# mokemokechicken/reversi-alpha-zero

Hardware: NVIDIA H100
Metric: self_play_games_per_sec (higher is better)
Workload: dtype f16

## Files before the change

### include/rz_engine.h

```cpp
#ifndef RZ_ENGINE_H
#define RZ_ENGINE_H

#include <stddef.h>
#include <stdint.h>

#ifdef __cplusplus
extern "C" {
#endif

#define RZ_OK 0
#define RZ_EINVAL (-1)
#define RZ_ECUDA (-2)
#define RZ_ENOMEM (-3)
#define RZ_ESTATE (-4)
#define RZ_ECAPACITY (-5)
#define RZ_EIO (-6)

#define RZ_ABI_VERSION 2

int rz_abi_version(void);
const char* rz_last_error(void);
int rz_device_count(int* count);


// ... 89 lines not shown
    int32_t start_rethinking_turn;
    int32_t allowed_resign_turn;
    int32_t use_resign_threshold;
    int32_t share_mtcs_info;
    int32_t eval_mode;
    int32_t net_impl;
    int32_t max_plies;
    int32_t warm_start;
    int32_t overlap_groups;
    int32_t max_sims_per_wave;
    int32_t use_solver_turn;
    int32_t use_solver_turn_in_simulation;
    int32_t reset_mtcs_info_per_game;
    int32_t max_searches_per_game;
    int32_t arena_simulation_num;
    float c_puct;
    float noise_eps;
    float dirichlet_alpha;
    float resign_threshold;
    float disable_resignation_rate;
    uint64_t seed;
    uint64_t first_game_id;
    uint64_t game_id_stride;
    uint64_t max_games;
} rz_engine_cfg;

typedef struct rz_ply {
    uint64_t own, enemy;
    int32_t n_visit[64];
    int16_t action;
// ... 22 lines not shown
    uint8_t pad[2];
    int32_t table_nodes;
    int32_t pad2;
} rz_game;

typedef struct rz_stats {
    uint64_t games_started, games_finished;
    uint64_t expansions;
    uint64_t simulations;
    uint64_t waves;
    uint64_t plies;
    uint64_t nn_launches, mcts_launches;
    uint64_t max_nodes_used, max_edges_used;
    double nn_ms, mcts_ms;
    double run_ms;
} rz_stats;

int rz_engine_create(const rz_engine_cfg* cfg, rz_net* net , int device,
                     rz_engine** out);
int rz_engine_destroy(rz_engine* e);
int rz_engine_run(rz_engine* e, uint64_t finished_target, uint64_t max_waves);
int rz_engine_poll(rz_engine* e, rz_game* games, size_t game_cap, size_t* n_games, rz_ply* plies, size_t ply_cap,
                   size_t* n_plies);
int rz_engine_stats(rz_engine* e, rz_stats* out);
int rz_engine_set_max_games(rz_engine* e, uint64_t max_games);
int rz_engine_set_warm_start_profile(rz_engine* e, const float* weight, int n);
int rz_engine_set_simulation_num(rz_engine* e, int32_t sims);
int rz_engine_set_second_net(rz_engine* e, rz_net* net_b, int enable);
int rz_engine_set_resign_threshold(rz_engine* e, int use_resign_threshold, float resign_threshold);
int rz_engine_search_root(rz_engine* e, uint64_t own, uint64_t enemy, int player, int slot, int keep_tree,
                          int32_t* n_visit, float* w_sum);

int rz_write_play_data(const char* path, const rz_game* games, size_t n_games, const rz_ply* plies,
                       int save_policy_of_tau_1, int change_tau_turn, size_t* n_records);

typedef struct rz_play_row {
    uint64_t own, enemy;
    int32_t n_visit[64];
    int32_t z;
// ... 78 lines not shown
```

### reversi-alpha-zero_b200/csrc/rz_engine.cu

```cuda
#include <deque>
#include <mutex>
#include <new>
#include <vector>
#include <stdlib.h>
#include <string.h>
#include "rz_bitboard.cuh"
#include "rz_net.cuh"
#include "rz_solver.cuh"

namespace rz {
namespace solver {
constexpr int kBlockThreads = 128;
__global__ void __launch_bounds__(kBlockThreads) solve_active_kernel(SolveCtx* __restrict__ ctx, const uint32_t* __restrict__ active,
                                                                     const uint32_t* __restrict__ n_active, uint32_t* __restrict__ next,
                                                                     uint32_t* __restrict__ n_next, u64* tt_base, long long budget_ns) {
    const uint32_t n = *n_active;
    if (n == 0) return;
    const uint32_t tid = blockIdx.x * blockDim.x + threadIdx.x, total = gridDim.x * blockDim.x, n_warps = total >> 5;
    const long long deadline = global_ns() + budget_ns;
    const TT tt{tt_base + (size_t)tid * kTtEntries * kTtWordsPerEntry};
    for (uint32_t r = (tid & 31u) * n_warps + (tid >> 5); r < n; r += total) {
        const uint32_t idx = active[r];
        if (!solve_advance(ctx + idx, tt, deadline)) next[atomicAdd(n_next, 1u)] = idx;
    }
// ... 57 lines not shown
    u64 games_played;
    uint32_t gen;
    uint32_t n_nodes, n_edges;
    uint32_t n_expand, n_rootsel, n_sims, sims_started, sims_target;
    uint32_t ply;
    uint8_t phase, tl, log_sel, enable_resign;
    uint8_t resigned_mask, search_only, n_pending, n_parked;
    uint8_t pending[kMaxK], parked[kMaxK];
    u64 root_own, root_enemy;
    uint8_t root_pid, black_net, cur_net;
    uint8_t root_req;
    uint32_t ply_waves;
    uint32_t n_solves, n_searched_plies;
};

struct Status {
    unsigned long long games_started, games_finished, expansions, simulations, plies, idle_slots;
    unsigned long long max_nodes, max_edges;
    int error;
    int pad;
};

struct DevCfg {
    int G, S, K, vl, change_tau_turn, thinking_loop, required_visit, start_rethinking_turn, allowed_resign_turn;
    int use_resign, share, max_plies, warm_start, sims_cap, two_nets, solver_turn, solver_sim_turn, keep_games;
    float c_puct, noise_eps, alpha, resign_threshold, disable_resignation_rate;
    u64 seed, first_game_id, game_id_stride, max_games;
    uint32_t nodes_cap, edges_cap, hash_cap;
    float warm_cdf[60];
    float warm_waves[60];
};

struct DevPtrs {
    Slot* slots;
    Descent* desc;
    uint32_t* hash;
    Node* nodes;
    Edge* edges;
    rz_ply* plies;
    rz_game* mail_hdr;
    uint8_t* mail_flag;
    Status* status;
    uint32_t* batch_count;
    u64* batch_own;
    u64* batch_enemy;
    float* policy;
    float* value;
    solver::SolveCtx* sctx;
    uint32_t* sactive;
    uint32_t* solve_count;
    float* keep_policy;
    float* keep_value;
    u64* solver_tt;
};

__device__ __forceinline__ uint32_t hash_key(u64 own, u64 enemy, uint32_t kpid) {
    u64 h = own * 0x9E3779B97F4A7C15ULL ^ (enemy + 0x7F4A7C15ULL) * 0xC2B2AE3D27D4EB4FULL ^ (u64)kpid * 0x165667B19E3779F9ULL;
    h ^= h >> 29; h *= 0xBF58476D1CE4E5B9ULL; h ^= h >> 32;
    return (uint32_t)h;
}

#include "rz_engine_warp.cuh"

__global__ void fake_eval_kernel(const u64* __restrict__ own, const u64* __restrict__ enemy, const uint32_t* __restrict__ count,
                                 float* __restrict__ policy, float* __restrict__ value, float sign) {
    const uint32_t n = *count;
    for (uint32_t i = blockIdx.x * blockDim.x + threadIdx.x; i < n * 64; i += gridDim.x * blockDim.x) {
        policy[i] = 1.0f / 64.0f;
        if ((i & 63) == 0) value[i >> 6] = sign * ((float)(popc64(own[i >> 6]) - popc64(enemy[i >> 6])) / 64.0f);
    }
}

__global__ void init_slots_kernel(const DevCfg c, const DevPtrs p) {
    const int s = blockIdx.x * blockDim.x + threadIdx.x;
    if (s >= c.G) return;
// ... 61 lines not shown
    size_t solver_tt_words_per_group;
    int solve_parity[2];
    long long solver_budget_ns;
    void* arena[32];
    int n_arena;
    Status* h_status;
    uint8_t* h_flags;
    uint64_t waves, nn_launches, mcts_launches;
    uint64_t finished_total;
    std::deque<FinishedGame> queue;
    std::mutex queue_mutex;
    cudaEvent_t ev[2 * 3 * 8];
    cudaEvent_t ev_run[3];
    int ev_used;
    double nn_ms, mcts_ms, run_ms;
};

static int collect_timing(rz_engine* e) {
    for (int g = 0; g < e->n_groups; ++g)
        for (int i = 0; i < e->ev_used; ++i) {
            float a = 0.f, b = 0.f;
            cudaEvent_t* ev = e->ev + (g * 8 + i) * 3;
            RZ_CUDA_TRY(cudaEventElapsedTime(&a, ev[0], ev[1]));
            RZ_CUDA_TRY(cudaEventElapsedTime(&b, ev[1], ev[2]));
            e->mcts_ms += a; e->nn_ms += b;
        }
    e->ev_used = 0;
    return RZ_OK;
}

static int dev_alloc(rz_engine* e, void** ptr, size_t bytes, bool zero) {
// ... 25 lines not shown
                                            cudaMemcpyDeviceToHost, e->stream));
        RZ_CUDA_TRY(cudaMemsetAsync(e->dp.mail_flag + i, 0, 1, e->stream));
        RZ_CUDA_TRY(cudaStreamSynchronize(e->stream));
        {
            std::lock_guard<std::mutex> lock(e->queue_mutex);
            e->queue.push_back(std::move(fg));
        }
        e->finished_total++;
    }
    return RZ_OK;
}

static int launch_wave(rz_engine* e) {
    const DevCfg& c = e->dc;
    const bool timed = e->ev_used < 8;
    for (int g = 0; g < e->n_groups; ++g) {
        cudaStream_t st = g == 0 ? e->stream : e->stream2;
        const int s0 = e->group_slot0[g], s1 = e->group_slot0[g + 1];
        cudaEvent_t* ev = e->ev + (g * 8 + e->ev_used) * 3;
        const size_t rows = (size_t)(s1 - s0) * c.K;
        if (timed) RZ_CUDA_TRY(cudaEventRecord(ev[0], st));
        for (int net = 0; net <= c.two_nets; ++net) RZ_CUDA_TRY(cudaMemsetAsync(e->dp.batch_count + (net * 2 + g) * 64, 0, sizeof(uint32_t), st));
        const bool solving = c.solver_turn > 0 || c.solver_sim_turn > 0;
        const int par = e->solve_parity[g];
        if (solving) RZ_CUDA_TRY(cudaMemsetAsync(e->dp.solve_count + (g * 2 + (1 - par)) * 64, 0, sizeof(uint32_t), st));
        tick_warp_kernel<<<(s1 - s0 + 1) / 2, kWarpTickThreads, 0, st>>>(c, e->dp, s0, s1, g, par);
        RZ_LAUNCH_CHECK();
        e->mcts_launches++;
        if (solving) {
            const size_t list = (size_t)c.G * (c.K + 1);
// ... 9 lines not shown
        for (int net = 0; net <= c.two_nets; ++net) {
            uint32_t* count = e->dp.batch_count + (net * 2 + g) * 64;
            const size_t row0 = (size_t)net * c.G * c.K + (size_t)s0 * c.K;
            if (e->cfg.eval_mode == RZ_EVAL_FAKE) {
                fake_eval_kernel<<<num_sms() * 4, 256, 0, st>>>(e->dp.batch_own + row0, e->dp.batch_enemy + row0, count, e->dp.policy + row0 * 64,
                                                              e->dp.value + row0, net ? -1.f : 1.f);
                RZ_LAUNCH_CHECK();
                e->mcts_launches++;
            } else {
                RZ_TRY(net_forward_counted(net ? e->net_b : e->net, e->dp.batch_own + row0, e->dp.batch_enemy + row0, e->dp.policy + row0 * 64,
                                           e->dp.value + row0, count, rows, e->cfg.net_impl, st));
                e->nn_launches++;
            }
        }
        if (timed) RZ_CUDA_TRY(cudaEventRecord(ev[2], st));
    }
    if (timed) e->ev_used++;
    e->waves++;
    return RZ_OK;
}

static int sync_all(rz_engine* e) {
    if (e->n_groups > 1) RZ_CUDA_TRY(cudaStreamSynchronize(e->stream2));
    RZ_CUDA_TRY(cudaStreamSynchronize(e->stream));
    return RZ_OK;
}

static int read_status(rz_engine* e) {
    RZ_TRY(sync_all(e));
    RZ_CUDA_TRY(cudaMemcpyAsync(e->h_status, e->dp.status, sizeof(Status), cudaMemcpyDeviceToHost, e->stream));
// ... 12 lines not shown
int rz_engine_create(const rz_engine_cfg* cfg, rz_net* net, int device, rz_engine** out) {
    RZ_REQUIRE(cfg && out, "rz_engine_create: null pointer");
    RZ_REQUIRE(cfg->games >= 1 && cfg->games <= (1 << 20), "games out of range (%d)", cfg->games);
    RZ_REQUIRE(cfg->simulation_num_per_move >= 1 && cfg->simulation_num_per_move <= 100000, "simulation_num_per_move out of range");
    RZ_REQUIRE(cfg->parallel_search_num >= 1 && cfg->parallel_search_num <= kMaxK, "parallel_search_num must be 1..%d", kMaxK);
    RZ_REQUIRE(cfg->thinking_loop >= 1 && cfg->thinking_loop <= 255, "thinking_loop must be 1..255");
    RZ_REQUIRE(cfg->eval_mode == RZ_EVAL_FAKE || net, "rz_engine_create: a network is required unless eval_mode == RZ_EVAL_FAKE");
    RZ_REQUIRE(cfg->game_id_stride >= 1, "game_id_stride must be >= 1");
    RZ_CUDA_TRY(cudaSetDevice(device));
    rz_engine* e = new (std::nothrow) rz_engine();
    if (!e) { set_error("out of host memory"); return RZ_ENOMEM; }
    e->cfg = *cfg; e->net = net; e->net_b = nullptr; e->device = device; e->n_arena = 0;
    e->waves = e->nn_launches = e->mcts_launches = e->finished_total = 0;
    e->h_status = nullptr; e->h_flags = nullptr; e->stream = nullptr; e->stream2 = nullptr;
    e->ev_used = 0; e->nn_ms = e->mcts_ms = e->run_ms = 0.0;
    for (int i = 0; i < 48; ++i) e->ev[i] = nullptr;
    e->ev_run[0] = e->ev_run[1] = e->ev_run[2] = nullptr;
    e->n_groups = cfg->overlap_groups == 1 ? 1 : (cfg->overlap_groups == 2 ? 2 : (cfg->games >= 256 ? 2 : 1));
    if (cfg->games < 2) e->n_groups = 1;
    e->group_slot0[0] = 0;
    e->group_slot0[1] = e->n_groups == 2 ? (cfg->games + 1) / 2 : cfg->games;
    e->group_slot0[2] = cfg->games;
    DevCfg& c = e->dc;
    c.G = cfg->games; c.S = cfg->simulation_num_per_move; c.K = cfg->parallel_search_num; c.vl = cfg->virtual_loss;
    c.change_tau_turn = cfg->change_tau_turn; c.thinking_loop = cfg->thinking_loop; c.required_visit = cfg->required_visit_to_decide_action;
    c.start_rethinking_turn = cfg->start_rethinking_turn; c.allowed_resign_turn = cfg->allowed_resign_turn;
    c.use_resign = cfg->use_resign_threshold; c.share = cfg->share_mtcs_info; c.max_plies = cfg->max_plies > 0 ? cfg->max_plies : 64;
    c.warm_start = cfg->warm_start;
    for (int t = 0; t < 60; ++t) { c.warm_cdf[t] = t < 58 ? (float)(t + 1) / 58.f : 1.f; c.warm_waves[t] = 0.f; }
    c.two_nets = 0;
// ... 23 lines not shown
    if (!rc) rc = dev_alloc(e, (void**)&p.desc, G * c.K * sizeof(Descent), true);
    if (!rc) rc = dev_alloc(e, (void**)&p.hash, G * c.hash_cap * sizeof(uint32_t), true);
    if (!rc) rc = dev_alloc(e, (void**)&p.nodes, G * c.nodes_cap * sizeof(Node), false);
    if (!rc) rc = dev_alloc(e, (void**)&p.edges, G * (size_t)c.edges_cap * sizeof(Edge), false);
    if (!rc) rc = dev_alloc(e, (void**)&p.plies, G * 2 * c.max_plies * sizeof(rz_ply), false);
    if (!rc) rc = dev_alloc(e, (void**)&p.mail_hdr, G * 2 * sizeof(rz_game), true);
    if (!rc) rc = dev_alloc(e, (void**)&p.mail_flag, G * 2, true);
    if (!rc) rc = dev_alloc(e, (void**)&p.status, sizeof(Status), true);
    if (!rc) rc = dev_alloc(e, (void**)&p.batch_count, 1024, true);
    if (!rc) rc = dev_alloc(e, (void**)&p.batch_own, (B + 2) * sizeof(u64), true);
    if (!rc) rc = dev_alloc(e, (void**)&p.batch_enemy, (B + 2) * sizeof(u64), true);
    if (!rc) rc = dev_alloc(e, (void**)&p.policy, (B + 2) * 64 * sizeof(float), true);
    if (!rc) rc = dev_alloc(e, (void**)&p.value, (B + 2) * sizeof(float), true);
    const bool solving = c.solver_turn > 0 || c.solver_sim_turn > 0;
    const size_t SR = G * (c.K + 1);
    if (!rc) rc = dev_alloc(e, (void**)&p.solve_count, 1024, true);
    p.sctx = nullptr; p.sactive = nullptr; p.keep_policy = nullptr; p.keep_value = nullptr; p.solver_tt = nullptr;
    e->solve_parity[0] = e->solve_parity[1] = 0;
    {
        const char* b = getenv("RZ_SOLVER_BUDGET_US");
        const long long us = b ? atoll(b) : 2000;
        e->solver_budget_ns = (us > 0 ? us : 2000) * 1000LL;
    }
    e->solver_tt_words_per_group = (size_t)num_sms() * solver::kBlockThreads * solver::kTtEntries * solver::kTtWordsPerEntry;
    if (solving) {
        if (!rc) rc = dev_alloc(e, (void**)&p.sctx, SR * sizeof(solver::SolveCtx), true);
        if (!rc) rc = dev_alloc(e, (void**)&p.sactive, 4 * SR * sizeof(uint32_t), true);
        if (!rc) rc = dev_alloc(e, (void**)&p.keep_policy, G * c.K * 64 * sizeof(float), true);
        if (!rc) rc = dev_alloc(e, (void**)&p.keep_value, G * c.K * sizeof(float), true);
        if (!rc) rc = dev_alloc(e, (void**)&p.solver_tt, e->solver_tt_words_per_group * 2 * sizeof(u64), true);
    }
    if (!rc && cudaMallocHost((void**)&e->h_status, sizeof(Status)) != cudaSuccess) { set_error("cudaMallocHost failed"); rc = RZ_ENOMEM; }
    if (!rc && cudaMallocHost((void**)&e->h_flags, G * 2) != cudaSuccess) { set_error("cudaMallocHost failed"); rc = RZ_ENOMEM; }
    for (int i = 0; i < 48 && !rc; ++i)
        if (cudaEventCreate(&e->ev[i]) != cudaSuccess) { set_error("cudaEventCreate failed"); rc = RZ_ECUDA; }
    for (int i = 0; i < 3 && !rc; ++i)
        if (cudaEventCreate(&e->ev_run[i]) != cudaSuccess) { set_error("cudaEventCreate failed"); rc = RZ_ECUDA; }
    if (rc) { rz_engine_destroy(e); return rc; }
    init_slots_kernel<<<(c.G + 127) / 128, 128, 0, e->stream>>>(c, p);
    ce = cudaStreamSynchronize(e->stream);
    if (ce != cudaSuccess) { set_error("rz_engine_create: %s", cudaGetErrorString(ce)); rz_engine_destroy(e); return RZ_ECUDA; }
    *out = e;
    return RZ_OK;
}

// ... 67 lines not shown
    return RZ_OK;
}

int rz_engine_stats(rz_engine* e, rz_stats* out) {
    RZ_REQUIRE(e && out, "rz_engine_stats: null pointer");
    RZ_CUDA_TRY(cudaSetDevice(e->device));
    RZ_TRY(sync_all(e));
    RZ_CUDA_TRY(cudaMemcpyAsync(e->h_status, e->dp.status, sizeof(Status), cudaMemcpyDeviceToHost, e->stream));
    RZ_CUDA_TRY(cudaStreamSynchronize(e->stream));
    const Status& s = *e->h_status;
    out->games_started = s.games_started; out->games_finished = s.games_finished; out->expansions = s.expansions;
    out->simulations = s.simulations; out->waves = e->waves; out->plies = s.plies; out->nn_launches = e->nn_launches;
    out->mcts_launches = e->mcts_launches; out->max_nodes_used = s.max_nodes; out->max_edges_used = s.max_edges;
    RZ_TRY(collect_timing(e));
    out->nn_ms = e->nn_ms; out->mcts_ms = e->mcts_ms; out->run_ms = e->run_ms;
    return RZ_OK;
}

int rz_engine_set_simulation_num(rz_engine* e, int32_t sims) {
    RZ_REQUIRE(e && sims >= 1, "rz_engine_set_simulation_num: bad argument");
    const uint64_t searches = e->cfg.max_searches_per_game > 0 ? (uint64_t)e->cfg.max_searches_per_game
                                                                  : (uint64_t)60 * (e->dc.thinking_loop > 2 ? 2 : e->dc.thinking_loop);
    uint64_t need = searches * sims * (uint64_t)e->dc.keep_games + 64;
    RZ_REQUIRE(need <= e->dc.nodes_cap, "simulation count %d exceeds the arenas sized at creation", sims);
    e->dc.S = sims;
    e->cfg.simulation_num_per_move = sims;
    return RZ_OK;
}

int rz_engine_set_max_games(rz_engine* e, uint64_t max_games) {
// ... 15 lines not shown
    double cum = 0.0;
    for (int t = 0; t < 60; ++t) {
        if (t < n) cum += weight[t];
        e->dc.warm_cdf[t] = t >= n - 1 ? 1.f : (float)(cum / total);
        e->dc.warm_waves[t] = t < n ? weight[t] : 0.f;
    }
    return RZ_OK;
}

int rz_engine_set_second_net(rz_engine* e, rz_net* net_b, int enable) {
    RZ_REQUIRE(e, "rz_engine_set_second_net: null engine");
    RZ_REQUIRE(!enable || e->cfg.eval_mode == RZ_EVAL_FAKE || net_b, "rz_engine_set_second_net: a second network is required");
    RZ_REQUIRE(e->waves == 0, "rz_engine_set_second_net: must be called before the first wave");
    e->net_b = enable ? net_b : nullptr;
    e->dc.two_nets = enable ? 1 : 0;
    return RZ_OK;
}

int rz_engine_set_resign_threshold(rz_engine* e, int use_resign_threshold, float resign_threshold) {
    RZ_REQUIRE(e, "rz_engine_set_resign_threshold: null engine");
    e->dc.use_resign = use_resign_threshold ? 1 : 0;
    e->dc.resign_threshold = resign_threshold;
    e->cfg.use_resign_threshold = e->dc.use_resign;
    e->cfg.resign_threshold = resign_threshold;
    return RZ_OK;
}

int rz_engine_search_root(rz_engine* e, uint64_t own, uint64_t enemy, int player, int slot, int keep_tree, int32_t* n_visit,
                          float* w_sum) {
    RZ_REQUIRE(e && n_visit && w_sum && (player == 1 || player == 2) && slot >= 0 && slot < e->dc.G, "rz_engine_search_root: bad argument");
// ... 25 lines not shown
```

### reversi-alpha-zero_b200/csrc/rz_engine_warp.cuh

```cuda
#pragma once

struct WCtx {
    const DevCfg& c;
    const DevPtrs& p;
    const int s, lane;
    Slot sl;
    uint8_t dstat[kMaxK];
    Descent* desc;
    uint32_t* hash;
    Node* nodes;
    Edge* edges;
    static constexpr unsigned kFull = 0xffffffffu;

    __device__ WCtx(const DevCfg& c_, const DevPtrs& p_, int s_, int lane_)
        : c(c_), p(p_), s(s_), lane(lane_), sl(p_.slots[s_]), desc(p_.desc + (size_t)s_ * c_.K), hash(p_.hash + (size_t)s_ * c_.hash_cap),
          nodes(p_.nodes + (size_t)s_ * c_.nodes_cap), edges(p_.edges + (size_t)s_ * c_.edges_cap) {
        for (int k = 0; k < kMaxK; ++k) dstat[k] = k < c_.K ? desc[k].status : (uint8_t)D_PENDING;
    }
    __device__ void write_back() {
        if (lane == 0) {
            p.slots[s] = sl;
            for (int k = 0; k < c.K; ++k) desc[k].status = dstat[k];
        }
        __syncwarp();
// ... 604 lines not shown
            if (sl.search_only) { sl.phase = PH_IDLE; if (lane == 0) atomicAdd(&p.status->idle_slots, 1ULL); break; }
            sl.phase = PH_DECIDE;
        } else if (sl.phase == PH_DECIDE) {
            x.decide();
        } else if (sl.phase == PH_NEWGAME) {
            if (p.mail_flag[(size_t)s * 2 + sl.log_sel]) break;
            x.new_game();
        } else {
            break;
        }
    }
    const int n_leaves = sl.phase == PH_SEARCH ? sl.n_pending : 0;
    const uint32_t root_req = (sl.phase == PH_SOLVE && sl.root_req) ? 1u : 0u;
    const bool mine = lane < n_leaves;
    const bool is_solve = mine && x.desc[sl.pending[mine ? lane : 0]].dihedral == kSolveMarker;
    const unsigned sv_mask = __ballot_sync(0xffffffffu, is_solve), nn_mask = __ballot_sync(0xffffffffu, mine && !is_solve);
    const uint32_t n_nn = __popc(nn_mask), n_sv = __popc(sv_mask) + root_req;
    const uint32_t net = c.two_nets ? sl.cur_net : 0u;
    uint32_t base = 0, sbase = 0;
    uint32_t* s_count = p.solve_count + (group * 2 + parity) * 64;
    uint32_t* s_list = p.sactive + (size_t)(group * 2 + parity) * c.G * (c.K + 1);
    if (lane == 0 && n_nn > 0) base = atomicAdd(p.batch_count + (net * 2 + group) * 64, n_nn);
    if (lane == 0 && n_sv > 0) sbase = atomicAdd(s_count, n_sv);
    base = __shfl_sync(0xffffffffu, base, 0);
    sbase = __shfl_sync(0xffffffffu, sbase, 0);
    if (root_req) sl.root_req = 0;
    x.write_back();
    const uint32_t below = (1u << lane) - 1u;
    if (mine && !is_solve) {
        Descent& d = x.desc[sl.pending[lane]];
        const uint32_t at = net * (uint32_t)c.G * (uint32_t)c.K + (uint32_t)slot0 * (uint32_t)c.K + base + __popc(nn_mask & below);
        d.leaf_index = at;
        d.kept = 0;
        p.batch_own[at] = dihedral(d.leaf_own, d.dihedral);
        p.batch_enemy[at] = dihedral(d.leaf_enemy, d.dihedral);
    } else if (is_solve) {
        const int di = sl.pending[lane];
        const Descent& d = x.desc[di];
        const uint32_t idx = (uint32_t)s * (uint32_t)(c.K + 1) + (uint32_t)di;
        solver::ctx_init(p.sctx + idx, d.leaf_own, d.leaf_enemy, 0);
        s_list[sbase + __popc(sv_mask & below)] = idx;
    }
    if (root_req && lane == 0) {
        const uint32_t idx = (uint32_t)s * (uint32_t)(c.K + 1) + (uint32_t)c.K;
        solver::ctx_init(p.sctx + idx, sl.root_own, sl.root_enemy, 1);
        s_list[sbase + (n_sv - 1)] = idx;
    }
}
```

### reversi-alpha-zero_b200/csrc/rz_net.cu

```cuda
#include <math.h>
#include <stdlib.h>
#include <string.h>
#include <new>
#include "rz_bitboard.cuh"
#include "rz_net.cuh"
#include "rz_tc_common.cuh"

namespace rz {

constexpr float kBnEps = 1e-3f;

__global__ void fold_bn_kernel(const float* __restrict__ blob, size_t group_off, size_t kernel_floats, int cout,
                               float* __restrict__ scale, float* __restrict__ shift) {
    int c = blockIdx.x * blockDim.x + threadIdx.x;
    if (c >= cout) return;
    const float* p = blob + group_off + kernel_floats;
    float bias = p[c], gamma = p[cout + c], beta = p[2 * cout + c], mean = p[3 * cout + c], var = p[4 * cout + c];
    float s = gamma / sqrtf(var + kBnEps);
    scale[c] = s;
    shift[c] = beta + (bias - mean) * s;
}

constexpr int kGThreads = 256;

// ... 179 lines not shown
    const int F = c.filters, L = n_conv_layers(c);
    float* ss = net->scale_shift;
    for (int l = 0; l < L; ++l) {
        const size_t off = l == 0 ? net->off_conv0 : net->off_res0 + (size_t)(l - 1) * net->res_stride_conv;
        const size_t kf = l == 0 ? (size_t)9 * 2 * F : (size_t)9 * F * F;
        fold_bn_kernel<<<(F + 127) / 128, 128, 0, stream>>>(net->blob, off, kf, F, ss + (size_t)l * 2 * F, ss + (size_t)l * 2 * F + F);
    }
    float* ssh = ss + (size_t)L * 2 * F;
    fold_bn_kernel<<<1, 32, 0, stream>>>(net->blob, net->off_policy_conv, (size_t)F * 2, 2, ssh, ssh + 2);
    fold_bn_kernel<<<1, 32, 0, stream>>>(net->blob, net->off_value_conv, (size_t)F, 1, ssh + 4, ssh + 5);
    RZ_LAUNCH_CHECK();
    if (F == 256) RZ_TRY(net_pack_tc(net, stream));
    else if (tc_width(F)) RZ_TRY(net_pack_tc_narrow(net, stream));
    RZ_CUDA_TRY(cudaStreamSynchronize(stream));
    net->loaded = true;
    return RZ_OK;
}

}

using namespace rz;

extern "C" {

int rz_net_create(const rz_net_cfg* cfg, int device, rz_net** out) {
    RZ_REQUIRE(cfg && out, "rz_net_create: null pointer");
    RZ_REQUIRE(cfg->kernel_size == 3, "only cnn_filter_size == 3 is supported (got %d)", cfg->kernel_size);
    RZ_REQUIRE(cfg->filters >= 2 && cfg->filters <= 256 && cfg->res_blocks >= 0 && cfg->res_blocks <= 64 && cfg->value_fc >= 1 &&
                   cfg->value_fc <= 4096,
               "unsupported model configuration (filters=%d res_blocks=%d value_fc=%d)", cfg->filters, cfg->res_blocks, cfg->value_fc);
// ... 153 lines not shown
```

### reversi-alpha-zero_b200/csrc/rz_net.cuh

```cuda
#pragma once
#include <cuda_fp16.h>
#include <mutex>
#include "rz_common.cuh"

struct rz_net {
    rz_net_cfg cfg;
    int device;
    bool loaded;
    size_t blob_floats;
    float* blob;
    float* scale_shift;
    size_t off_conv0, off_res0, res_stride_conv;
    size_t off_policy_conv, off_policy_fc_k, off_policy_fc_b;
    size_t off_value_conv, off_value_fc1_k, off_value_fc1_b, off_value_fc2_k, off_value_fc2_b;
    __half* tc_w0;
    __half* tc_w;
    float* res;
    cudaEvent_t res_done;
    float* feat;
    size_t feat_rows;
    void* scratch;
    size_t scratch_bytes;
};

// ... 34 lines not shown
```

### reversi-alpha-zero_b200/reversi_zero_b200/_cabi.py

```python
import ctypes as C
import os

_HERE = os.path.dirname(os.path.abspath(__file__))
LIB_PATH = os.path.join(os.path.dirname(_HERE), "csrc", "librz_engine.so")

u64p, u8p, i8p, f32p, i32p = (C.POINTER(C.c_uint64), C.POINTER(C.c_uint8), C.POINTER(C.c_int8),
                              C.POINTER(C.c_float), C.POINTER(C.c_int32))
vp, sz = C.c_void_p, C.c_size_t


class RzError(RuntimeError):
    pass


class EnvState(C.Structure):
    _fields_ = [("black", C.c_uint64), ("white", C.c_uint64), ("next_player", C.c_uint8), ("turn", C.c_uint8),
                ("done", C.c_uint8), ("winner", C.c_uint8)]


class NetCfg(C.Structure):
    _fields_ = [("filters", C.c_int32), ("res_blocks", C.c_int32), ("value_fc", C.c_int32), ("kernel_size", C.c_int32)]


class TrainCfg(C.Structure):
    _fields_ = [("max_batch", C.c_int32), ("momentum", C.c_float), ("l2_reg", C.c_float), ("bn_momentum", C.c_float)]


class EngineCfg(C.Structure):
    _fields_ = [(n, C.c_int32) for n in (
        "games", "simulation_num_per_move", "parallel_search_num", "virtual_loss", "change_tau_turn", "thinking_loop",
        "required_visit_to_decide_action", "start_rethinking_turn", "allowed_resign_turn", "use_resign_threshold",
        "share_mtcs_info", "eval_mode", "net_impl", "max_plies", "warm_start", "overlap_groups", "max_sims_per_wave", "use_solver_turn", "use_solver_turn_in_simulation",
        "reset_mtcs_info_per_game", "max_searches_per_game", "arena_simulation_num")] + [(n, C.c_float) for n in (
            "c_puct", "noise_eps", "dirichlet_alpha", "resign_threshold", "disable_resignation_rate")] + [
        (n, C.c_uint64) for n in ("seed", "first_game_id", "game_id_stride", "max_games")]


class Ply(C.Structure):
    _fields_ = [("own", C.c_uint64), ("enemy", C.c_uint64), ("n_visit", C.c_int32 * 64), ("action", C.c_int16),
                ("player", C.c_uint8), ("loops", C.c_uint8), ("recorded", C.c_uint8), ("pad", C.c_uint8), ("waves", C.c_uint16),
                ("n", C.c_float), ("q", C.c_float)]


class Game(C.Structure):
    _fields_ = [("game_id", C.c_uint64), ("black", C.c_uint64), ("white", C.c_uint64), ("first_ply", C.c_int32),
                ("n_plies", C.c_int32), ("expansions", C.c_int32), ("simulations", C.c_int32), ("winner", C.c_uint8),
                ("black_z", C.c_int8), ("resign_enabled", C.c_uint8), ("resigned_mask", C.c_uint8), ("turn", C.c_uint8),
                ("black_net", C.c_uint8), ("pad", C.c_uint8 * 2), ("table_nodes", C.c_int32), ("pad2", C.c_int32)]


class PlayRow(C.Structure):
    _fields_ = [("own", C.c_uint64), ("enemy", C.c_uint64), ("n_visit", C.c_int32 * 64), ("z", C.c_int32), ("pad", C.c_int32)]


class DeepSolveStats(C.Structure):
    _fields_ = [("probes", C.c_int32), ("slices", C.c_int32), ("resplits", C.c_int32), ("pad", C.c_int32),
                ("leaves", C.c_int64), ("node_steps", C.c_int64), ("seconds", C.c_double)]


class Stats(C.Structure):
    _fields_ = [(n, C.c_uint64) for n in ("games_started", "games_finished", "expansions", "simulations", "waves",
                                          "plies", "nn_launches", "mcts_launches", "max_nodes_used", "max_edges_used")] + [
        ("nn_ms", C.c_double), ("mcts_ms", C.c_double), ("run_ms", C.c_double)]


SIGNATURES = {
    "rz_abi_version": (C.c_int, []),
    "rz_last_error": (C.c_char_p, []),
    "rz_device_count": (C.c_int, [C.POINTER(C.c_int)]),
    "rz_bitsliced_host": (C.c_int, [u8p, u64p, u64p, u64p, sz]),
    "rz_find_correct_moves_dev": (C.c_int, [vp, vp, vp, sz, vp]),
    "rz_find_correct_moves": (C.c_int, [u64p, u64p, u64p, sz]),
    "rz_calc_flip_dev": (C.c_int, [vp, vp, vp, vp, sz, vp]),
    "rz_calc_flip": (C.c_int, [u8p, u64p, u64p, u64p, sz]),
    "rz_step_dev": (C.c_int, [vp, vp, vp, vp, vp, vp, vp, vp, sz, vp]),
    "rz_step": (C.c_int, [u64p, u64p, u8p, u8p, u8p, u8p, i8p, u64p, sz]),
    "rz_dihedral_dev": (C.c_int, [vp, vp, vp, sz, vp]),
    "rz_solve_dev": (C.c_int, [vp, vp, vp, vp, vp, sz, vp]),
# ... 12 lines not shown
    "rz_net_load_weights": (C.c_int, [vp, f32p, sz]),
    "rz_net_load_weights_dev": (C.c_int, [vp, vp, sz, vp]),
    "rz_net_predict_dev": (C.c_int, [vp, vp, vp, vp, vp, sz, C.c_int, vp]),
    "rz_net_predict_counted_dev": (C.c_int, [vp, vp, vp, vp, vp, vp, sz, C.c_int, vp]),
    "rz_net_set_tower_cluster": (C.c_int, [C.c_int]),
    "rz_net_debug_tower_dev": (C.c_int, [vp, vp, vp, vp, vp, vp, sz, vp]),
    "rz_net_debug_heads_dev": (C.c_int, [vp, vp, vp, vp, vp, vp, vp, vp, sz, vp]),
    "rz_net_debug_heads_impl_dev": (C.c_int, [vp, vp, vp, vp, vp, vp, vp, vp, sz, C.c_int, vp]),
    "rz_net_select_impl": (C.c_int, [vp, sz, C.POINTER(C.c_int)]),
    "rz_net_predict": (C.c_int, [vp, u8p, f32p, f32p, sz, C.c_int]),
    "rz_engine_create": (C.c_int, [C.POINTER(EngineCfg), vp, C.c_int, C.POINTER(vp)]),
    "rz_engine_destroy": (C.c_int, [vp]),
    "rz_engine_run": (C.c_int, [vp, C.c_uint64, C.c_uint64]),
    "rz_engine_poll": (C.c_int, [vp, C.POINTER(Game), sz, C.POINTER(sz), C.POINTER(Ply), sz, C.POINTER(sz)]),
    "rz_engine_stats": (C.c_int, [vp, C.POINTER(Stats)]),
    "rz_engine_set_simulation_num": (C.c_int, [vp, C.c_int32]),
    "rz_engine_set_warm_start_profile": (C.c_int, [vp, f32p, C.c_int]),
    "rz_engine_set_max_games": (C.c_int, [vp, C.c_uint64]),
    "rz_engine_set_second_net": (C.c_int, [vp, vp, C.c_int]),
    "rz_engine_set_resign_threshold": (C.c_int, [vp, C.c_int, C.c_float]),
    "rz_engine_search_root": (C.c_int, [vp, C.c_uint64, C.c_uint64, C.c_int, C.c_int, C.c_int, i32p, f32p]),
    "rz_write_play_data": (C.c_int, [C.c_char_p, C.POINTER(Game), sz, C.POINTER(Ply), C.c_int, C.c_int, C.POINTER(sz)]),
    "rz_write_play_rows": (C.c_int, [C.c_char_p, C.POINTER(Game), sz, C.POINTER(Ply), C.c_int, C.c_int, C.POINTER(sz)]),
    "rz_read_play_rows": (C.c_int, [C.c_char_p, vp, sz, C.POINTER(sz), C.POINTER(C.c_int), C.POINTER(C.c_int)]),
    "rz_ingest_dev": (C.c_int, [vp, sz, C.c_int, C.c_int, vp, vp, vp, vp]),
    "rz_ingest": (C.c_int, [vp, sz, C.c_int, C.c_int, u8p, f32p, f32p]),
    "rz_ingest_json_dev": (C.c_int, [vp, sz, sz, vp, vp, vp, C.POINTER(sz), C.POINTER(sz), vp]),
    "rz_ingest_json_host": (C.c_int, [vp, sz, sz, vp, vp, vp, C.POINTER(sz), C.POINTER(sz)]),
    "rz_ingest_json": (C.c_int, [C.c_char_p, sz, vp, vp, vp, C.POINTER(sz), C.POINTER(sz)]),
    "rz_trainer_create": (C.c_int, [C.POINTER(NetCfg), C.POINTER(TrainCfg), C.c_int, C.POINTER(vp)]),
# ... 38 lines not shown
```

### reversi-alpha-zero_b200/reversi_zero_b200/engine.py

```python
import ctypes as C
import math

import numpy as np

from . import _cabi

EVAL_NET, EVAL_FAKE = 0, 1


def engine_cfg_from_play_config(pc, pdc=None, games=1024, seed=0, eval_mode=EVAL_NET, net_impl=0, first_game_id=0,
                                game_id_stride=1, max_games=0, warm_start=False, overlap_groups=0,
                                max_searches_per_game=0, use_solver=True, arena_simulation_num=0):
    cfg = _cabi.EngineCfg()
    cfg.games = games
    cfg.simulation_num_per_move = int(pc.simulation_num_per_move)
    cfg.parallel_search_num = int(pc.parallel_search_num)
    cfg.virtual_loss = int(pc.virtual_loss)
    cfg.change_tau_turn = int(pc.change_tau_turn)
    cfg.thinking_loop = int(pc.thinking_loop)
    cfg.required_visit_to_decide_action = int(pc.required_visit_to_decide_action)
    cfg.start_rethinking_turn = int(pc.start_rethinking_turn)
    cfg.allowed_resign_turn = int(pc.allowed_resign_turn)
    cfg.use_resign_threshold = 0 if pc.resign_threshold is None else 1
    cfg.share_mtcs_info = 1 if pc.share_mtcs_info_in_self_play else 0
    cfg.eval_mode = eval_mode
    cfg.net_impl = net_impl
    cfg.max_plies = 64
    cfg.warm_start = 1 if warm_start else 0
    cfg.overlap_groups = overlap_groups
    cfg.max_searches_per_game = max_searches_per_game
    cfg.arena_simulation_num = int(arena_simulation_num or 0)
    cfg.max_sims_per_wave = int(getattr(pc, "max_sims_per_wave", 0) or 0)
    cfg.reset_mtcs_info_per_game = int(getattr(pc, "reset_mtcs_info_per_game", 1) or 1) if cfg.share_mtcs_info else 1
    cfg.use_solver_turn = int(getattr(pc, "use_solver_turn", 0) or 0) if use_solver else 0
    cfg.use_solver_turn_in_simulation = int(getattr(pc, "use_solver_turn_in_simulation", 0) or 0) if use_solver else 0
    cfg.c_puct = float(pc.c_puct)
    cfg.noise_eps = float(pc.noise_eps)
    cfg.dirichlet_alpha = float(pc.dirichlet_alpha)
    cfg.resign_threshold = 0.0 if pc.resign_threshold is None else float(pc.resign_threshold)
    cfg.disable_resignation_rate = float(pc.disable_resignation_rate)
    cfg.seed = seed
    cfg.first_game_id = first_game_id
    cfg.game_id_stride = game_id_stride
    cfg.max_games = max_games
    return cfg

# ... 30 lines not shown
                    p = plies[j]
                    pl.append(dict(own=int(p.own), enemy=int(p.enemy), N=np.array(p.n_visit[:], dtype=np.int64), action=int(p.action),
                                   pid=int(p.player), loops=int(p.loops), recorded=bool(p.recorded), n=float(p.n), q=float(p.q),
                                   waves=int(p.waves)))
                out.append(dict(game_id=int(g.game_id), black=int(g.black), white=int(g.white), winner=int(g.winner),
                                black_z=int(g.black_z), expansions=int(g.expansions), simulations=int(g.simulations),
                                resign_enabled=bool(g.resign_enabled), resigned_mask=int(g.resigned_mask), turn=int(g.turn),
                                black_net=int(g.black_net), table_nodes=int(g.table_nodes), plies=pl))
        return out

    def stats(self):
        s = _cabi.Stats()
        _cabi.check(_cabi.lib().rz_engine_stats(self._h, C.byref(s)), "rz_engine_stats")
        return {n: (float if t is C.c_double else int)(getattr(s, n)) for n, t in _cabi.Stats._fields_}

    def set_simulation_num(self, sims):
        _cabi.check(_cabi.lib().rz_engine_set_simulation_num(self._h, int(sims)), "rz_engine_set_simulation_num")

    def set_max_games(self, n):
        _cabi.check(_cabi.lib().rz_engine_set_max_games(self._h, int(n)), "rz_engine_set_max_games")

    def set_warm_start_profile(self, weights):
        w = np.ascontiguousarray(weights, dtype=np.float32)
        _cabi.check(_cabi.lib().rz_engine_set_warm_start_profile(self._h, w.ctypes.data_as(_cabi.f32p), int(w.size)),
                    "rz_engine_set_warm_start_profile")

    def set_second_net(self, net_b=None, enable=True):
        self.net_b = net_b
        _cabi.check(_cabi.lib().rz_engine_set_second_net(self._h, net_b.handle if net_b is not None else None, int(bool(enable))),
                    "rz_engine_set_second_net")
# ... 31 lines not shown
```

Before: 22.50.

## Add device-side evaluation cache keyed by board position to skip NN inference

Adds a set-associative GPU hash table (2 GB by default) that stores the network's policy and value for each evaluated canonical board. MCTS leaf collection probes it and marks hits as already kept, so only misses go into the NN batch. After each wave an insert kernel writes the new results into the table, and a generation tag tied to the weights version invalidates old entries when weights are reloaded. This saves network evaluations for repeated positions across games, at the cost of lookup and insert kernels, seqlock atomics, per-turn stat counters and a large memory allocation.

```diff
diff --git a/include/rz_engine.h b/include/rz_engine.h
--- a/include/rz_engine.h
+++ b/include/rz_engine.h
@@ -127,6 +127,7 @@
     int32_t reset_mtcs_info_per_game;
     int32_t max_searches_per_game;
     int32_t arena_simulation_num;
+    int32_t eval_cache_mb;
     float c_puct;
     float noise_eps;
     float dirichlet_alpha;
@@ -179,6 +180,10 @@
     uint64_t max_nodes_used, max_edges_used;
     double nn_ms, mcts_ms;
     double run_ms;
+    uint64_t tower_rows;
+    uint64_t cache_lookups;
+    uint64_t cache_hits;
+    uint64_t cache_repeats;
 } rz_stats;
 
 int rz_engine_create(const rz_engine_cfg* cfg, rz_net* net , int device,
@@ -188,6 +193,7 @@
 int rz_engine_poll(rz_engine* e, rz_game* games, size_t game_cap, size_t* n_games, rz_ply* plies, size_t ply_cap,
                    size_t* n_plies);
 int rz_engine_stats(rz_engine* e, rz_stats* out);
+int rz_engine_cache_turn_stats(rz_engine* e, uint64_t* lookups, uint64_t* hits, int n);
 int rz_engine_set_max_games(rz_engine* e, uint64_t max_games);
 int rz_engine_set_warm_start_profile(rz_engine* e, const float* weight, int n);
 int rz_engine_set_simulation_num(rz_engine* e, int32_t sims);
diff --git a/reversi-alpha-zero_b200/csrc/rz_engine.cu b/reversi-alpha-zero_b200/csrc/rz_engine.cu
--- a/reversi-alpha-zero_b200/csrc/rz_engine.cu
+++ b/reversi-alpha-zero_b200/csrc/rz_engine.cu
@@ -95,11 +95,15 @@
     uint32_t n_solves, n_searched_plies;
 };
 
+constexpr int kCacheTurnBuckets = 61;
+
 struct Status {
     unsigned long long games_started, games_finished, expansions, simulations, plies, idle_slots;
     unsigned long long max_nodes, max_edges;
     int error;
     int pad;
+    unsigned long long tower_rows, cache_repeats;
+    unsigned long long cache_lookups[kCacheTurnBuckets], cache_hits[kCacheTurnBuckets];
 };
 
 struct DevCfg {
@@ -111,6 +115,14 @@
     float warm_cdf[60];
     float warm_waves[60];
 };
+
+__device__ __forceinline__ uint32_t hash_key(u64 own, u64 enemy, uint32_t kpid) {
+    u64 h = own * 0x9E3779B97F4A7C15ULL ^ (enemy + 0x7F4A7C15ULL) * 0xC2B2AE3D27D4EB4FULL ^ (u64)kpid * 0x165667B19E3779F9ULL;
+    h ^= h >> 29; h *= 0xBF58476D1CE4E5B9ULL; h ^= h >> 32;
+    return (uint32_t)h;
+}
+
+#include "rz_eval_cache.cuh"
 
 struct DevPtrs {
     Slot* slots;
@@ -133,13 +145,8 @@
     float* keep_policy;
     float* keep_value;
     u64* solver_tt;
-};
-
-__device__ __forceinline__ uint32_t hash_key(u64 own, u64 enemy, uint32_t kpid) {
-    u64 h = own * 0x9E3779B97F4A7C15ULL ^ (enemy + 0x7F4A7C15ULL) * 0xC2B2AE3D27D4EB4FULL ^ (u64)kpid * 0x165667B19E3779F9ULL;
-    h ^= h >> 29; h *= 0xBF58476D1CE4E5B9ULL; h ^= h >> 32;
-    return (uint32_t)h;
-}
+    EvalCache cache;
+};
 
 #include "rz_engine_warp.cuh"
 
@@ -231,7 +238,10 @@
     cudaEvent_t ev_run[3];
     int ev_used;
     double nn_ms, mcts_ms, run_ms;
-};
+    uint32_t cache_sets;
+};
+
+constexpr int64_t kDefaultEvalCacheMb = 2048;
 
 static int collect_timing(rz_engine* e) {
     for (int g = 0; g < e->n_groups; ++g)
@@ -287,6 +297,7 @@
 static int launch_wave(rz_engine* e) {
     const DevCfg& c = e->dc;
     const bool timed = e->ev_used < 8;
+    if (e->dp.cache.n_sets) e->dp.cache.gen = (uint32_t)e->net->weights_version;
     for (int g = 0; g < e->n_groups; ++g) {
         cudaStream_t st = g == 0 ? e->stream : e->stream2;
         const int s0 = e->group_slot0[g], s1 = e->group_slot0[g + 1];
@@ -326,6 +337,13 @@
             }
         }
         if (timed) RZ_CUDA_TRY(cudaEventRecord(ev[2], st));
+        if (e->dp.cache.n_sets) {
+            cache_insert_kernel<<<num_sms() * 2, 256, 0, st>>>(e->dp.cache, e->dp.batch_own + (size_t)s0 * c.K, e->dp.batch_enemy + (size_t)s0 * c.K,
+                                                              e->dp.policy + (size_t)s0 * c.K * 64, e->dp.value + (size_t)s0 * c.K,
+                                                              e->dp.batch_count + g * 64, &e->dp.status->cache_repeats);
+            RZ_LAUNCH_CHECK();
+            e->mcts_launches++;
+        }
     }
     if (timed) e->ev_used++;
     e->waves++;
@@ -368,6 +386,7 @@
     e->waves = e->nn_launches = e->mcts_launches = e->finished_total = 0;
     e->h_status = nullptr; e->h_flags = nullptr; e->stream = nullptr; e->stream2 = nullptr;
     e->ev_used = 0; e->nn_ms = e->mcts_ms = e->run_ms = 0.0;
+    e->cache_sets = 0;
     for (int i = 0; i < 48; ++i) e->ev[i] = nullptr;
     e->ev_run[0] = e->ev_run[1] = e->ev_run[2] = nullptr;
     e->n_groups = cfg->overlap_groups == 1 ? 1 : (cfg->overlap_groups == 2 ? 2 : (cfg->games >= 256 ? 2 : 1));
@@ -421,6 +440,21 @@
     if (!rc) rc = dev_alloc(e, (void**)&p.value, (B + 2) * sizeof(float), true);
     const bool solving = c.solver_turn > 0 || c.solver_sim_turn > 0;
     const size_t SR = G * (c.K + 1);
+    int64_t cache_mb = cfg->eval_cache_mb;
+    if (cache_mb == 0) {
+        const char* env = getenv("RZ_EVAL_CACHE_MB");
+        cache_mb = env ? atoll(env) : kDefaultEvalCacheMb;
+    }
+    if (cfg->eval_mode != RZ_EVAL_NET) cache_mb = 0;
+    const size_t cache_sets = cache_mb > 0 ? (size_t)cache_mb * 1048576 / (kCacheWays * sizeof(EvalCacheEntry)) : 0;
+    p.cache.entries = nullptr; p.cache.next = nullptr; p.cache.n_sets = 0; p.cache.gen = 0;
+    if (!rc && cache_sets >= 0xFFFFFFFFull / kCacheWays) { set_error("eval_cache_mb too large (%lld)", (long long)cache_mb); rc = RZ_EINVAL; }
+    if (!rc && cache_sets) {
+        if (!rc) rc = dev_alloc(e, (void**)&p.cache.entries, cache_sets * kCacheWays * sizeof(EvalCacheEntry), true);
+        if (!rc) rc = dev_alloc(e, (void**)&p.cache.next, cache_sets * sizeof(uint32_t), true);
+        e->cache_sets = (uint32_t)cache_sets;
+        p.cache.n_sets = e->cache_sets;
+    }
     if (!rc) rc = dev_alloc(e, (void**)&p.solve_count, 1024, true);
     p.sctx = nullptr; p.sactive = nullptr; p.keep_policy = nullptr; p.keep_value = nullptr; p.solver_tt = nullptr;
     e->solve_parity[0] = e->solve_parity[1] = 0;
@@ -433,9 +467,11 @@
     if (solving) {
         if (!rc) rc = dev_alloc(e, (void**)&p.sctx, SR * sizeof(solver::SolveCtx), true);
         if (!rc) rc = dev_alloc(e, (void**)&p.sactive, 4 * SR * sizeof(uint32_t), true);
+        if (!rc) rc = dev_alloc(e, (void**)&p.solver_tt, e->solver_tt_words_per_group * 2 * sizeof(u64), true);
+    }
+    if (solving || cache_sets) {
         if (!rc) rc = dev_alloc(e, (void**)&p.keep_policy, G * c.K * 64 * sizeof(float), true);
         if (!rc) rc = dev_alloc(e, (void**)&p.keep_value, G * c.K * sizeof(float), true);
-        if (!rc) rc = dev_alloc(e, (void**)&p.solver_tt, e->solver_tt_words_per_group * 2 * sizeof(u64), true);
     }
     if (!rc && cudaMallocHost((void**)&e->h_status, sizeof(Status)) != cudaSuccess) { set_error("cudaMallocHost failed"); rc = RZ_ENOMEM; }
     if (!rc && cudaMallocHost((void**)&e->h_flags, G * 2) != cudaSuccess) { set_error("cudaMallocHost failed"); rc = RZ_ENOMEM; }
@@ -533,6 +569,19 @@
     out->mcts_launches = e->mcts_launches; out->max_nodes_used = s.max_nodes; out->max_edges_used = s.max_edges;
     RZ_TRY(collect_timing(e));
     out->nn_ms = e->nn_ms; out->mcts_ms = e->mcts_ms; out->run_ms = e->run_ms;
+    out->tower_rows = s.tower_rows; out->cache_repeats = s.cache_repeats;
+    out->cache_lookups = out->cache_hits = 0;
+    for (int b = 0; b < kCacheTurnBuckets; ++b) { out->cache_lookups += s.cache_lookups[b]; out->cache_hits += s.cache_hits[b]; }
+    return RZ_OK;
+}
+
+int rz_engine_cache_turn_stats(rz_engine* e, uint64_t* lookups, uint64_t* hits, int n) {
+    RZ_REQUIRE(e && lookups && hits && n == kCacheTurnBuckets, "rz_engine_cache_turn_stats: bad argument");
+    RZ_CUDA_TRY(cudaSetDevice(e->device));
+    RZ_TRY(sync_all(e));
+    RZ_CUDA_TRY(cudaMemcpyAsync(e->h_status, e->dp.status, sizeof(Status), cudaMemcpyDeviceToHost, e->stream));
+    RZ_CUDA_TRY(cudaStreamSynchronize(e->stream));
+    for (int b = 0; b < n; ++b) { lookups[b] = e->h_status->cache_lookups[b]; hits[b] = e->h_status->cache_hits[b]; }
     return RZ_OK;
 }
 
@@ -578,6 +627,7 @@
     RZ_REQUIRE(e->waves == 0, "rz_engine_set_second_net: must be called before the first wave");
     e->net_b = enable ? net_b : nullptr;
     e->dc.two_nets = enable ? 1 : 0;
+    e->dp.cache.n_sets = enable ? 0u : e->cache_sets;
     return RZ_OK;
 }
 
diff --git a/reversi-alpha-zero_b200/csrc/rz_engine_warp.cuh b/reversi-alpha-zero_b200/csrc/rz_engine_warp.cuh
--- a/reversi-alpha-zero_b200/csrc/rz_engine_warp.cuh
+++ b/reversi-alpha-zero_b200/csrc/rz_engine_warp.cuh
@@ -642,8 +642,30 @@
     const uint32_t root_req = (sl.phase == PH_SOLVE && sl.root_req) ? 1u : 0u;
     const bool mine = lane < n_leaves;
     const bool is_solve = mine && x.desc[sl.pending[mine ? lane : 0]].dihedral == kSolveMarker;
-    const unsigned sv_mask = __ballot_sync(0xffffffffu, is_solve), nn_mask = __ballot_sync(0xffffffffu, mine && !is_solve);
+    const bool is_leaf = mine && !is_solve;
+    u64 t_own = 0, t_enemy = 0;
+    bool hit = false;
+    if (is_leaf) {
+        const Descent& d = x.desc[sl.pending[lane]];
+        t_own = dihedral(d.leaf_own, d.dihedral);
+        t_enemy = dihedral(d.leaf_enemy, d.dihedral);
+        if (p.cache.n_sets) {
+            const size_t row = (size_t)s * c.K + sl.pending[lane];
+            hit = cache_lookup(p.cache, t_own, t_enemy, p.keep_policy + row * 64, p.keep_value + row);
+        }
+    }
+    const unsigned sv_mask = __ballot_sync(0xffffffffu, is_solve), nn_mask = __ballot_sync(0xffffffffu, is_leaf && !hit);
     const uint32_t n_nn = __popc(nn_mask), n_sv = __popc(sv_mask) + root_req;
+    const uint32_t n_hit = __popc(__ballot_sync(0xffffffffu, hit));
+    if (lane == 0 && n_nn + n_hit > 0) {
+        if (p.cache.n_sets) {
+            const int turn = popc64(sl.root_own | sl.root_enemy) - 4;
+            const int b = (c.warm_start && sl.games_played == 1) ? kCacheTurnBuckets - 1 : (turn < 0 ? 0 : (turn > 59 ? 59 : turn));
+            atomicAdd(&p.status->cache_lookups[b], (unsigned long long)(n_nn + n_hit));
+            if (n_hit) atomicAdd(&p.status->cache_hits[b], (unsigned long long)n_hit);
+        }
+        if (n_nn) atomicAdd(&p.status->tower_rows, (unsigned long long)n_nn);
+    }
     const uint32_t net = c.two_nets ? sl.cur_net : 0u;
     uint32_t base = 0, sbase = 0;
     uint32_t* s_count = p.solve_count + (group * 2 + parity) * 64;
@@ -655,13 +677,15 @@
     if (root_req) sl.root_req = 0;
     x.write_back();
     const uint32_t below = (1u << lane) - 1u;
-    if (mine && !is_solve) {
+    if (hit) {
+        x.desc[sl.pending[lane]].kept = 1;
+    } else if (is_leaf) {
         Descent& d = x.desc[sl.pending[lane]];
         const uint32_t at = net * (uint32_t)c.G * (uint32_t)c.K + (uint32_t)slot0 * (uint32_t)c.K + base + __popc(nn_mask & below);
         d.leaf_index = at;
         d.kept = 0;
-        p.batch_own[at] = dihedral(d.leaf_own, d.dihedral);
-        p.batch_enemy[at] = dihedral(d.leaf_enemy, d.dihedral);
+        p.batch_own[at] = t_own;
+        p.batch_enemy[at] = t_enemy;
     } else if (is_solve) {
         const int di = sl.pending[lane];
         const Descent& d = x.desc[di];
diff --git a/reversi-alpha-zero_b200/csrc/rz_eval_cache.cuh b/reversi-alpha-zero_b200/csrc/rz_eval_cache.cuh
--- /dev/null
+++ b/reversi-alpha-zero_b200/csrc/rz_eval_cache.cuh
@@ -0,0 +1,86 @@
+#pragma once
+
+constexpr int kCacheWays = 8;
+
+struct __align__(16) EvalCacheEntry {
+    u64 own, enemy;
+    uint32_t seq;
+    uint32_t gen;
+    float value;
+    uint32_t pad;
+    float policy[64];
+};
+static_assert(sizeof(EvalCacheEntry) == 288, "cache entry layout");
+
+struct EvalCache {
+    EvalCacheEntry* entries;
+    uint32_t* next;
+    uint32_t n_sets;
+    uint32_t gen;
+};
+
+__device__ __forceinline__ EvalCacheEntry* cache_set(const EvalCache& t, u64 own, u64 enemy) {
+    return t.entries + (size_t)(hash_key(own, enemy, 0) % t.n_sets) * kCacheWays;
+}
+
+__device__ __forceinline__ uint32_t volatile_load(const uint32_t* p) { return *(const volatile uint32_t*)p; }
+
+__device__ bool cache_lookup(const EvalCache& t, u64 own, u64 enemy, float* policy_out, float* value_out) {
+    EvalCacheEntry* set = cache_set(t, own, enemy);
+    int way = -1;
+#pragma unroll
+    for (int w = 0; w < kCacheWays; ++w) {
+        const ulonglong2 k = __ldcg(reinterpret_cast<const ulonglong2*>(set + w));
+        const uint2 m = __ldcg(reinterpret_cast<const uint2*>(&set[w].seq));
+        if (k.x == own && k.y == enemy && m.y == t.gen && !(m.x & 1u)) way = w;
+    }
+    if (way < 0) return false;
+    EvalCacheEntry* e = set + way;
+    const uint32_t s1 = volatile_load(&e->seq);
+    __threadfence();
+    const ulonglong2 k = __ldcg(reinterpret_cast<const ulonglong2*>(e));
+    const uint32_t g = __ldcg(&e->gen);
+    const float v = __ldcg(&e->value);
+    const float4* src = reinterpret_cast<const float4*>(e->policy);
+    float4* dst = reinterpret_cast<float4*>(policy_out);
+#pragma unroll
+    for (int i = 0; i < 16; ++i) dst[i] = __ldcg(src + i);
+    __threadfence();
+    const uint32_t s2 = volatile_load(&e->seq);
+    if (s1 != s2 || (s1 & 1u) || k.x != own || k.y != enemy || g != t.gen) return false;
+    *value_out = v;
+    return true;
+}
+
+__global__ void cache_insert_kernel(const EvalCache t, const u64* __restrict__ own, const u64* __restrict__ enemy,
+                                    const float* __restrict__ policy, const float* __restrict__ value,
+                                    const uint32_t* __restrict__ count, unsigned long long* repeats) {
+    const uint32_t n = *count;
+    for (uint32_t r = blockIdx.x * blockDim.x + threadIdx.x; r < n; r += gridDim.x * blockDim.x) {
+        const u64 o = own[r], en = enemy[r];
+        EvalCacheEntry* set = cache_set(t, o, en);
+        bool present = false;
+#pragma unroll
+        for (int w = 0; w < kCacheWays; ++w) {
+            const ulonglong2 k = __ldcg(reinterpret_cast<const ulonglong2*>(set + w));
+            const uint32_t g = __ldcg(&set[w].gen);
+            if (k.x == o && k.y == en && g == t.gen) present = true;
+        }
+        const unsigned rep = __ballot_sync(__activemask(), present);
+        if (present) {
+            if ((threadIdx.x & 31) == (unsigned)(__ffs(rep) - 1)) atomicAdd(repeats, (unsigned long long)__popc(rep));
+            continue;
+        }
+        EvalCacheEntry* e = set + atomicAdd(t.next + (set - t.entries) / kCacheWays, 1u) % kCacheWays;
+        const uint32_t s = volatile_load(&e->seq);
+        if ((s & 1u) || atomicCAS(&e->seq, s, s + 1u) != s) continue;
+        __threadfence();
+        e->own = o; e->enemy = en; e->gen = t.gen; e->value = value[r];
+        const float4* src = reinterpret_cast<const float4*>(policy + (size_t)r * 64);
+        float4* dst = reinterpret_cast<float4*>(e->policy);
+#pragma unroll
+        for (int i = 0; i < 16; ++i) dst[i] = src[i];
+        __threadfence();
+        atomicExch(&e->seq, s + 2u);
+    }
+}
diff --git a/reversi-alpha-zero_b200/csrc/rz_net.cu b/reversi-alpha-zero_b200/csrc/rz_net.cu
--- a/reversi-alpha-zero_b200/csrc/rz_net.cu
+++ b/reversi-alpha-zero_b200/csrc/rz_net.cu
@@ -217,6 +217,7 @@
     else if (tc_width(F)) RZ_TRY(net_pack_tc_narrow(net, stream));
     RZ_CUDA_TRY(cudaStreamSynchronize(stream));
     net->loaded = true;
+    net->weights_version++;
     return RZ_OK;
 }
 
diff --git a/reversi-alpha-zero_b200/csrc/rz_net.cuh b/reversi-alpha-zero_b200/csrc/rz_net.cuh
--- a/reversi-alpha-zero_b200/csrc/rz_net.cuh
+++ b/reversi-alpha-zero_b200/csrc/rz_net.cuh
@@ -7,6 +7,7 @@
     rz_net_cfg cfg;
     int device;
     bool loaded;
+    uint64_t weights_version;
     size_t blob_floats;
     float* blob;
     float* scale_shift;
diff --git a/reversi-alpha-zero_b200/reversi_zero_b200/_cabi.py b/reversi-alpha-zero_b200/reversi_zero_b200/_cabi.py
--- a/reversi-alpha-zero_b200/reversi_zero_b200/_cabi.py
+++ b/reversi-alpha-zero_b200/reversi_zero_b200/_cabi.py
@@ -31,7 +31,7 @@
         "games", "simulation_num_per_move", "parallel_search_num", "virtual_loss", "change_tau_turn", "thinking_loop",
         "required_visit_to_decide_action", "start_rethinking_turn", "allowed_resign_turn", "use_resign_threshold",
         "share_mtcs_info", "eval_mode", "net_impl", "max_plies", "warm_start", "overlap_groups", "max_sims_per_wave", "use_solver_turn", "use_solver_turn_in_simulation",
-        "reset_mtcs_info_per_game", "max_searches_per_game", "arena_simulation_num")] + [(n, C.c_float) for n in (
+        "reset_mtcs_info_per_game", "max_searches_per_game", "arena_simulation_num", "eval_cache_mb")] + [(n, C.c_float) for n in (
             "c_puct", "noise_eps", "dirichlet_alpha", "resign_threshold", "disable_resignation_rate")] + [
         (n, C.c_uint64) for n in ("seed", "first_game_id", "game_id_stride", "max_games")]
 
@@ -61,7 +61,8 @@
 class Stats(C.Structure):
     _fields_ = [(n, C.c_uint64) for n in ("games_started", "games_finished", "expansions", "simulations", "waves",
                                           "plies", "nn_launches", "mcts_launches", "max_nodes_used", "max_edges_used")] + [
-        ("nn_ms", C.c_double), ("mcts_ms", C.c_double), ("run_ms", C.c_double)]
+        ("nn_ms", C.c_double), ("mcts_ms", C.c_double), ("run_ms", C.c_double)] + [
+        (n, C.c_uint64) for n in ("tower_rows", "cache_lookups", "cache_hits", "cache_repeats")]
 
 
 SIGNATURES = {
@@ -104,6 +105,7 @@
     "rz_engine_run": (C.c_int, [vp, C.c_uint64, C.c_uint64]),
     "rz_engine_poll": (C.c_int, [vp, C.POINTER(Game), sz, C.POINTER(sz), C.POINTER(Ply), sz, C.POINTER(sz)]),
     "rz_engine_stats": (C.c_int, [vp, C.POINTER(Stats)]),
+    "rz_engine_cache_turn_stats": (C.c_int, [vp, u64p, u64p, C.c_int]),
     "rz_engine_set_simulation_num": (C.c_int, [vp, C.c_int32]),
     "rz_engine_set_warm_start_profile": (C.c_int, [vp, f32p, C.c_int]),
     "rz_engine_set_max_games": (C.c_int, [vp, C.c_uint64]),
diff --git a/reversi-alpha-zero_b200/reversi_zero_b200/engine.py b/reversi-alpha-zero_b200/reversi_zero_b200/engine.py
--- a/reversi-alpha-zero_b200/reversi_zero_b200/engine.py
+++ b/reversi-alpha-zero_b200/reversi_zero_b200/engine.py
@@ -10,7 +10,7 @@
 
 def engine_cfg_from_play_config(pc, pdc=None, games=1024, seed=0, eval_mode=EVAL_NET, net_impl=0, first_game_id=0,
                                 game_id_stride=1, max_games=0, warm_start=False, overlap_groups=0,
-                                max_searches_per_game=0, use_solver=True, arena_simulation_num=0):
+                                max_searches_per_game=0, use_solver=True, arena_simulation_num=0, eval_cache_mb=0):
     cfg = _cabi.EngineCfg()
     cfg.games = games
     cfg.simulation_num_per_move = int(pc.simulation_num_per_move)
@@ -30,6 +30,7 @@
     cfg.overlap_groups = overlap_groups
     cfg.max_searches_per_game = max_searches_per_game
     cfg.arena_simulation_num = int(arena_simulation_num or 0)
+    cfg.eval_cache_mb = int(eval_cache_mb)
     cfg.max_sims_per_wave = int(getattr(pc, "max_sims_per_wave", 0) or 0)
     cfg.reset_mtcs_info_per_game = int(getattr(pc, "reset_mtcs_info_per_game", 1) or 1) if cfg.share_mtcs_info else 1
     cfg.use_solver_turn = int(getattr(pc, "use_solver_turn", 0) or 0) if use_solver else 0
@@ -90,6 +91,12 @@
         _cabi.check(_cabi.lib().rz_engine_stats(self._h, C.byref(s)), "rz_engine_stats")
         return {n: (float if t is C.c_double else int)(getattr(s, n)) for n, t in _cabi.Stats._fields_}
 
+    def cache_turn_stats(self):
+        lookups, hits = np.zeros(61, np.uint64), np.zeros(61, np.uint64)
+        _cabi.check(_cabi.lib().rz_engine_cache_turn_stats(self._h, lookups.ctypes.data_as(_cabi.u64p), hits.ctypes.data_as(_cabi.u64p), 61),
+                    "rz_engine_cache_turn_stats")
+        return lookups, hits
+
     def set_simulation_num(self, sims):
         _cabi.check(_cabi.lib().rz_engine_set_simulation_num(self._h, int(sims)), "rz_engine_set_simulation_num")
 
```

Result: faster. 24.70, median of 6 (+9.8%).
